# libAudioFlux/audioFlux

Measured on AMD Instinct MI355X. Metric: audio frames/sec (mel+MFCC, n_fft=2048 hop=512), higher is better.
Workload: dtype f32

## Files before the change

### audioflux_amd/csrc/hip/afx_melfused.hip

```cpp
#include <hip/hip_runtime.h>

#include <cstdlib>

#include "afx_melplan.h"

namespace {

const AfxMelSize *size_of(int radix2Exp) {
    switch (radix2Exp) {
        case 9: return afx_mel_size512();
        case 10: return afx_mel_size1k();
        case 11: return afx_mel_size2k();
        case 12: return afx_mel_size4k();
        default: return nullptr;
    }
}

void pack_band(const AfxBandPlan *band, int TA, int WP, float *wL, int *meta) {
    for (int l = 0; l < 64; ++l) {
        for (int t = 0; t < band->tapsA; ++t) wL[(size_t)l * WP + t] = band->wA[(size_t)t * 64 + l];
        for (int t = 0; t < band->tapsB; ++t) wL[(size_t)l * WP + TA + t] = band->wB[(size_t)t * 64 + l];
        meta[l] = band->startA[l];
        meta[64 + l] = band->startB[l];
        meta[128 + l] = band->rowA[l];
        meta[192 + l] = band->rowB[l];
        meta[256 + l] = (int)band->segIdx[l];
        meta[320 + l] = (int)band->segIdx[64 + l];
    }
}

}

extern "C" int afxk_melfused_variant(int radix2Exp, int tapsA, int tapsB) {
    const AfxMelSize *s = size_of(radix2Exp);
    if (afxdev_no_fused() || !s) return -1;
    for (int i = 0; i < s->numVariants; ++i)
        if (tapsA <= s->variants[i].tapsA && tapsB <= s->variants[i].tapsB) return i;
    return -1;
}

extern "C" int afxk_melfused_kind(const void *plan) {
    const AfxMelPlan *p = static_cast<const AfxMelPlan *>(plan);
    return !p ? 0 : size_of(p->radix2Exp)->kindBase + (p->split ? 2 : 1);
}

extern "C" void afxk_melfused_destroy(void *plan) {
    AfxMelPlan *p = static_cast<AfxMelPlan *>(plan);
    if (!p) return;
    afxdev_free(p->dTab);
    afxdev_free(p->dMeta);
    free(p);
}

extern "C" int afxk_melfused_create(void **plan, int radix2Exp, const float *hWindow,
                                    const AfxBandPlan *band, void *stream) {
    *plan = nullptr;
    const int variant = afxk_melfused_variant(radix2Exp, band->tapsA, band->tapsB);
    if (variant < 0) return AFX_ERR_UNSUPPORTED;
    const AfxMelSize *s = size_of(radix2Exp);
    const int TA = s->variants[variant].tapsA, TB = s->variants[variant].tapsB;
    const int WP = TA + TB + 4;
    const size_t bytes = (size_t)s->bandOff + (size_t)64 * WP * 4;
    AfxMelPlan *p = static_cast<AfxMelPlan *>(calloc(1, sizeof(AfxMelPlan)));
    float *tab = static_cast<float *>(calloc(bytes, 1));
    if (!p || !tab) {
        free(p);
        free(tab);
        return AFX_ERR_NOMEM;
    }
    p->radix2Exp = radix2Exp;
    p->variant = variant;
    p->num = band->num;
    p->split = band->split;
    s->fill(tab, hWindow);
    int meta[384];
    pack_band(band, TA, WP, tab + s->bandOff / 4, meta);
    int st = afxdev_malloc(reinterpret_cast<void **>(&p->dTab), bytes);
    if (st == AFX_OK) st = afxdev_h2d(p->dTab, tab, bytes, stream);
    if (st == AFX_OK) st = afxdev_malloc(reinterpret_cast<void **>(&p->dMeta), sizeof(meta));
    if (st == AFX_OK) st = afxdev_h2d(p->dMeta, meta, sizeof(meta), stream);
    if (st == AFX_OK) st = afxdev_stream_sync(stream);
    free(tab);
    if (st != AFX_OK) {
        afxk_melfused_destroy(p);
        return st;
    }
    *plan = p;
    return AFX_OK;
}

extern "C" int afxk_melfused_run(void *plan, const AfxMelFusedArgs *a, void *stream) {
    const AfxMelPlan *p = static_cast<const AfxMelPlan *>(plan);
    if (!p) return AFX_ERR_ARG;
    if (a->energy && p->radix2Exp != 11) return AFX_ERR_UNSUPPORTED;
    if (a->specMap > 4) return AFX_ERR_ARG;
    return size_of(p->radix2Exp)->run(p, a, stream);
}
```

### audioflux_amd/csrc/hip/afx_melfused2.hip

```cpp
#include <hip/hip_runtime.h>

#include <cmath>
#include <cstdlib>
#include <cstring>

#include "afx_melplan.h"
#include "afx_melparts.h"
#include "afx_ccblock.h"

#ifdef AFX_V2_NTIN
#define AFX_V2_LOAD(p) __builtin_nontemporal_load(p)
#define AFX_V2_NT true
#else
#define AFX_V2_LOAD(p) (*(p))
#define AFX_V2_NT false
#endif
#ifndef AFX_V2_CCEVERY
#define AFX_V2_CCEVERY 16
#endif
#ifdef AFX_V2_STAMPS
#include <cstdio>
#include <vector>
#endif

namespace {

constexpr int NFFT = 2048;
constexpr int MC = 1024;
constexpr int WAVES = 12;
constexpr int WAVES_CPLX = 12;
__host__ __device__ constexpr int waves_of(bool cplx) { return cplx ? WAVES_CPLX : WAVES; }
constexpr int P1 = 72;
constexpr int PROW_OFF = 5120;
constexpr int PROW_F = 1104;
constexpr int WAVE_LDS = PROW_OFF + PROW_F * 4;
constexpr int CLAIM_LDS = 16;
static_assert(16 * P1 * 8 <= PROW_OFF + 1025 * 4, "exchange image must end before the zero pad");
constexpr int T_WIN = 0;
constexpr int T_TW1 = 8192;
constexpr int T_TW2 = 16384;
constexpr int TW2_PITCH = 144;
constexpr int T_TW3 = 16960;
constexpr int T_BAND = 21056;
__host__ __device__ constexpr int wpitch(int ta, int tb) { return ta + tb + 4; }
__host__ __device__ constexpr int tab_bytes(int ta, int tb) { return T_BAND + 64 * wpitch(ta, tb) * 4; }
constexpr int DCT_PITCH = 36;
__host__ __device__ constexpr int block_lds_bytes(int ta, int tb, bool cc) {
    return tab_bytes(ta, tb) + (cc ? 64 * DCT_PITCH * 4 : 0) + WAVES * WAVE_LDS + CLAIM_LDS;
}

__host__ __device__ constexpr int claim_length(int left, int waves, int minRun) {
    const int g = left / (2 * waves);
    if (left >= 16 * waves) return g >= 16 ? g & ~15 : 16;
    return (g & ~3) > minRun ? g & ~3 : minRun;
}

struct KArgs2 {
    const float *x;
    long long clipStride;
    long long totalFrames;
    int timeLength, hop;
    long long framesPerWg;
    int aligned;
    const float4 *tab;
    const int *meta;
    int specMap, postPow;
    float normValue;
    float *out;
    float *outIm;
    int num;
    const float *dct;
    int ccNum, ccCbrt;
    float *cc;
    float *energy, *rms, *zcr;
    const float *win;
    int binLo, binCount;
    long long outPitch;
    int vecOut;
#ifdef AFX_V2_STAMPS
    unsigned long long *stamps;
#endif
};
#ifdef AFX_V2_STAMPS
constexpr int STAMP_WORDS = 64, STAMP_HEAD = 8;
#endif


#ifndef AFX_PRIO_MASK
#define AFX_PRIO_MASK 0x1E
#endif
#ifndef AFX_PRIO_LEVEL
#define AFX_PRIO_LEVEL 1
#endif
#define MEL_PHASE(p)                                                                                       \
    do {                                                                                                   \
        if (AFX_PRIO_MASK != 0) __builtin_amdgcn_s_setprio(((AFX_PRIO_MASK >> (p)) & 1) ? AFX_PRIO_LEVEL : 0); \
    } while (0)

__device__ __forceinline__ float wave_sum(float v) {
#pragma unroll
    for (int o = 32; o > 0; o >>= 1) v += __shfl_xor(v, o, 64);
    return v;
}

template <int TA, int TB, int SHIFT, bool SPLIT, int CC, bool TEMPORAL, bool CPLX = false, bool STFT = false>
__global__ __launch_bounds__(waves_of(CPLX) * 64, 3) void k_stft_mel_v2(KArgs2 a) {
    constexpr int NWV = waves_of(CPLX);
    static_assert(!(CPLX && (CC || TEMPORAL)), "complex results: the bank only");
    static_assert(!STFT || (TA == 0 && TB == 0 && !SPLIT && CC == 0 && !TEMPORAL && !CPLX), "STFT instantiations: real rows, no bank");
    extern __shared__ __attribute__((aligned(16))) unsigned char smem[];
    const int lane = threadIdx.x & 63;
    const int wave = threadIdx.x >> 6;
    constexpr int WP = wpitch(TA, TB);
    constexpr int TABB = tab_bytes(TA, TB);
    constexpr int DCTB = CC == 1 ? 64 * DCT_PITCH * 4 : 0;
    unsigned char *wreg = smem + TABB + DCTB + wave * WAVE_LDS;
    float *prow = reinterpret_cast<float *>(wreg + PROW_OFF);

    {
        float4 *s4 = reinterpret_cast<float4 *>(smem);
        for (int i = threadIdx.x + (STFT ? T_TW1 / 16 : 0); i < TABB / 16; i += NWV * 64) s4[i] = a.tab[i];
        if constexpr (STFT) {
            v2 *tw = reinterpret_cast<v2 *>(smem + T_WIN);
            const v2 *w2 = reinterpret_cast<const v2 *>(a.win);
            for (int at = threadIdx.x; at < 1024; at += NWV * 64) {
                const int n1 = 2 * (at >> 7) + (at & 1), l = (at & 127) >> 1;
                tw[at] = w2[64 * n1 + l];
            }
        }
        if constexpr (CC == 1) {
            float *tabD = reinterpret_cast<float *>(smem + TABB);
            for (int i = threadIdx.x; i < 64 * 32; i += NWV * 64) {
                const int l = i >> 5, e = i & 31;
                const int fi = l & 15, g = l >> 4;
                tabD[l * DCT_PITCH + e] =
                    fi < a.ccNum ? a.dct[(long long)fi * a.num + 16 * (e >> 2) + 4 * g + (e & 3)] : 0.f;
            }
        }
        for (int i = 1025 + lane; i < PROW_F; i += 64) prow[i] = 0.f;
        if (threadIdx.x == 0) *reinterpret_cast<int *>(smem + TABB + DCTB + NWV * WAVE_LDS) = 0;
    }
    __syncthreads();

    const int k1 = lane >> 2, m2 = lane & 3;
    const unsigned T0 = lds_addr(smem), W0 = lds_addr(wreg);
    const unsigned aWin = T0 + T_WIN + 16 * lane;
    const unsigned aTw2 = T0 + T_TW2 + TW2_PITCH * m2;
    const unsigned aE1w = W0 + 8 * (8 * (k1 >> 1) + 2 * m2 + (k1 & 1));
    const unsigned aE1r = W0 + 576 * k1 + 16 * m2;
    const unsigned aE2w = W0 + 32 * k1 + 16 * ((m2 >> 1) ^ ((k1 >> 3) & 1)) + 8 * (m2 & 1);
    const int b3l = (lane >> 3) & 1;
    const unsigned aAlo = W0 + 32 * lane + 16 * b3l, aAhi = W0 + 32 * lane + 16 * (1 - b3l);
    const int qm0 = lane == 0 ? 128 : 256 - lane, qm1 = 192 - lane;
    const unsigned aB0lo = W0 + 32 * qm0 + 16 * ((qm0 >> 3) & 1), aB0hi = W0 + 32 * qm0 + 16 * (1 - ((qm0 >> 3) & 1));
    const unsigned aB1lo = W0 + 32 * qm1 + 16 * ((qm1 >> 3) & 1), aB1hi = W0 + 32 * qm1 + 16 * (1 - ((qm1 >> 3) & 1));
    const unsigned aT3lo = T0 + T_TW3 + 32 * lane + 16 * b3l, aT3hi = T0 + T_TW3 + 32 * lane + 16 * (1 - b3l);
    const unsigned R = W0 + PROW_OFF;
    const unsigned aP01 = R + 4 * lane;
    const unsigned aP23 = R + 4 * (lane == 0 ? 128 : lane + 512);
    const unsigned aQs1 = R + 4 * (192 - lane);
    const unsigned aQ23 = R + 4 * (lane == 0 ? 640 : 256 - lane);
    const bool lane0 = (lane == 0);

    const int startA = STFT ? 0 : a.meta[lane], startB = STFT ? 0 : a.meta[64 + lane];
    const int rowA = STFT ? -1 : a.meta[128 + lane], rowB = STFT ? -1 : a.meta[192 + lane];
    const unsigned seg0 = SPLIT ? (unsigned)a.meta[256 + lane] : 0u, seg1 = SPLIT ? (unsigned)a.meta[320 + lane] : 0u;
    const unsigned apa = R + 4 * startA, apb = R + 4 * startB;
    const unsigned awr = T0 + T_BAND + 4 * WP * lane;
    const unsigned vRaw = 8u * (unsigned)lane, vLane = 4u * (unsigned)lane;
    const bool okA = rowA >= 0, okB = rowB >= 0;
    const unsigned vRowA = okA ? 4u * (unsigned)rowA : 0u, vRowB = okB ? 4u * (unsigned)rowB : 0u;
    const long long rowPitch = STFT ? a.outPitch : (long long)a.num;

    const long long wgBeg = (long long)blockIdx.x * a.framesPerWg;
    const int wgN = (int)(a.totalFrames - wgBeg < a.framesPerWg ? a.totalFrames - wgBeg : a.framesPerWg);
    const int minRun = wgN >= 4 * NWV ? 4 : wgN > NWV ? (wgN + NWV - 1) / NWV : 1;
    int *claimed = reinterpret_cast<int *>(smem + TABB + DCTB + NWV * WAVE_LDS);
    const int wgClip = (int)(wgBeg / a.timeLength);
    const unsigned wgT = (unsigned)(wgBeg - (long long)wgClip * a.timeLength);
    auto locate = [&](long long fr, int &c, int &tt) {
        const unsigned at = wgT + (unsigned)(fr - wgBeg);
        c = wgClip + (int)(at / (unsigned)a.timeLength);
        tt = (int)(at % (unsigned)a.timeLength);
    };
    auto claim = [&](long long &rb, long long &re) -> bool {
        int s = wgN, l = 0;
        if (lane0) {
            const int left = wgN - __atomic_load_n(claimed, __ATOMIC_RELAXED);
            if (left > 0) {
                l = claim_length(left, NWV, minRun);
                s = __atomic_fetch_add(claimed, l, __ATOMIC_RELAXED);
            }
        }
        s = __builtin_amdgcn_readfirstlane(s);
        l = __builtin_amdgcn_readfirstlane(l);
        if (s >= wgN) return false;
        rb = wgBeg + s;
        re = wgBeg + (s + l < wgN ? s + l : wgN);
        return true;
    };
    int ccN = 0;
#ifdef AFX_V2_STAMPS
    unsigned long long *stamp = a.stamps + ((long long)blockIdx.x * NWV + wave) * STAMP_WORDS;
    int stampN = 0;
// ... 272 lines not shown
                    split_pair(A1, B1, hi2(wlo[s]), pk[s][1], pq[s][1]);
                    split_pair(A2, B2, lo2(whi[s]), pk[s][2], pq[s][2]);
                    split_pair(A3, B3, hi2(whi[s]), pk[s][3], pq[s][3]);
                }
            }
        }
        if constexpr (CPLX) {
            WR2ST_32(aP01 - PROW_OFF, ik[0][0], ik[0][1], 0, 4);
            WR2ST_32(aP23 - PROW_OFF, ik[0][2], ik[0][3], 0, 4);
            WR2ST_32(aP01 - PROW_OFF, ik[1][0], ik[1][1], 1, 5);
            WR2ST_32(aP01 - PROW_OFF, ik[1][2], ik[1][3], 9, 13);
            WR2ST_32(aQs1 - PROW_OFF, iq[0][1], iq[0][0], 9, 13);
            WR2ST_32(aQ23 - PROW_OFF, iq[0][3], iq[0][2], 0, 4);
            WR2ST_32(aQs1 - PROW_OFF, iq[1][3], iq[1][2], 0, 4);
            WR2ST_32(aQs1 - PROW_OFF, iq[1][1], iq[1][0], 8, 12);
            float *prowI = reinterpret_cast<float *>(wreg);
            if (lane0) prowI[512] = i512;
            prowI[1025 + lane] = 0.f;
            if (lane < PROW_F - 1025 - 64) prowI[1025 + 64 + lane] = 0.f;
        }
        WR2ST_32_S(4, aP01, pk[0][0], pk[0][1], 0, 4);
        WR2ST_32_S(4, aP23, pk[0][2], pk[0][3], 0, 4);
        WR2ST_32_S(4, aP01, pk[1][0], pk[1][1], 1, 5);
        WR2ST_32_S(4, aP01, pk[1][2], pk[1][3], 9, 13);
        WR2ST_32_S(4, aQs1, pq[0][1], pq[0][0], 9, 13);
        WR2ST_32_S(4, aQ23, pq[0][3], pq[0][2], 0, 4);
        WR2ST_32_S(4, aQs1, pq[1][3], pq[1][2], 0, 4);
        WR2ST_32_S(4, aQs1, pq[1][1], pq[1][0], 8, 12);
        if (lane0) prow[512] = p512;
        wave_lds_sync();
#pragma unroll
        for (int pass = 0; pass < (CPLX ? 2 : 1); ++pass) {
        const unsigned bpa = (CPLX && pass) ? apa - PROW_OFF : apa, bpb = (CPLX && pass) ? apb - PROW_OFF : apb;
        if (!CPLX && a.specMap) {
            for (int k = lane; k < 1025; k += 64) {
                const float p = prow[k];
                prow[k] = a.specMap == 1 ? sqrtf(p) : powf(p, a.normValue);
            }
            wave_lds_sync();
        }

        if constexpr (STFT) {
            MEL_PHASE(6);
            raw_landed();
            float *orow = a.out + rowOff;
            if (a.vecOut) {
                const float4 *p4 = reinterpret_cast<const float4 *>(prow);
                float4 *o4 = reinterpret_cast<float4 *>(orow);
                float4 q[4];
#pragma unroll
                for (int i = 0; i < 4; ++i) q[i] = p4[lane + 64 * i];
#pragma unroll
                for (int i = 0; i < 4; ++i) o4[lane + 64 * i] = q[i];
                if (lane0) o4[256] = p4[256];
            } else {
                for (int k = lane; k < a.binCount; k += 64) orow[k] = prow[a.binLo + k];
            }
        } else {
        MEL_PHASE(5);
        float accA, accB;
        {
            v2 sA, sB;
            band_stage<TA, TB, 4, CPLX>(awr, bpa, bpb, sA, sB);
            accA = sA.x + sA.y;
            accB = sB.x + sB.y;
        }
        if (!CPLX && !SPLIT && a.postPow) {
            accA = powf(accA, a.normValue);
            accB = powf(accB, a.normValue);
        }
        MEL_PHASE(6);
        if (pass == 0) raw_landed();
        if constexpr (CC != 0 && !SPLIT) {
            if (ccN == AFX_V2_CCEVERY) cc_block(f - AFX_V2_CCEVERY, (rowOff >> 7) - AFX_V2_CCEVERY, AFX_V2_CCEVERY);
        }
        float *const srow = ((CPLX && pass) ? a.outIm : a.out) + rowOff;
        if constexpr (SPLIT) {
            float *part = reinterpret_cast<float *>(wreg + (CPLX ? PROW_F * 4 : 0));
            static_assert(PROW_F * 4 + 129 * 4 <= PROW_OFF, "segment sums must fit between the two rows");
            part[lane] = accA;
            part[64 + lane] = accB;
            if (lane0) part[128] = 0.f;
            wave_lds_sync();
#pragma unroll
            for (int h = 0; h < 2; ++h) {
                const unsigned u = h ? seg1 : seg0;
                float sum = part[u & 255u] + part[(u >> 8) & 255u];
                sum += part[(u >> 16) & 255u];
                sum += part[u >> 24];
                if (!CPLX && a.postPow) sum = powf(sum, a.normValue);
                if (lane + 64 * h < a.num) GST32_S(vLane, sum, srow + 64 * h);
            }
        } else {
            if (okA) GST32_S(vRowA, accA, srow);
            if (okB) GST32_S(vRowB, accB, srow);
        }
        if constexpr (CC != 0) {
            ++ccN;
            if (f + 1 == fEnd || (SPLIT && ccN == 16)) cc_block(f + 1 - ccN, (rowOff >> 7) + 1 - ccN, ccN);
        }
        }
        wave_lds_sync();

        }

#ifdef AFX_V2_STAMPS
        ++stampN;
        if (lane0 && (stampN & 15) == 0 && STAMP_HEAD + (stampN >> 4) <= STAMP_WORDS) stamp[STAMP_HEAD - 1 + (stampN >> 4)] = __builtin_amdgcn_s_memtime();
#endif
        rowOff += rowPitch;
        if (++t == a.timeLength) {
            t = 0;
            ++clip;
        }
    }
    }
#ifdef AFX_V2_STAMPS
    if (lane0) {
        stamp[1] = __builtin_amdgcn_s_memtime();
        stamp[3] = (unsigned long long)stampN;
    }
#endif
}

void fill_tables(float *tab, const float *hWindow) {
    const double PI = 3.14159265358979323846;
    float *win = tab + T_WIN / 4, *tw1 = tab + T_TW1 / 4, *tw2 = tab + T_TW2 / 4, *tw3 = tab + T_TW3 / 4;
    for (int n1 = 0; n1 < 16; ++n1)
// ... 33 lines not shown
    const int asked = e ? atoi(e) : 0;
    const int cus = asked > 0 ? asked : afx_cu_count();
    long long fpw;
    long long blocks = afx_frame_split(total, cus, waves, 1, &fpw);
    *framesPerWg = fpw * waves;
    if (*framesPerWg > (1ll << 30)) {
        *framesPerWg = 1ll << 30;
        blocks = (total + *framesPerWg - 1) / *framesPerWg;
    }
    return blocks;
}

#ifdef AFX_V2_STAMPS
unsigned long long *stamps_begin(long long blocks, int waves) {
    unsigned long long *d = nullptr;
    const size_t n = (size_t)blocks * waves * STAMP_WORDS * 8;
    if (hipMalloc(&d, n) != hipSuccess || hipMemset(d, 0, n) != hipSuccess) return nullptr;
    return d;
}
void stamps_end(unsigned long long *d, long long blocks, int waves, void *stream) {
    const size_t n = (size_t)blocks * waves * STAMP_WORDS;
    std::vector<unsigned long long> h(n);
    (void)hipStreamSynchronize((hipStream_t)stream);
    if (hipMemcpy(h.data(), d, n * 8, hipMemcpyDeviceToHost) == hipSuccess)
        if (const char *name = getenv("AFX_V2_STAMPS_FILE"))
            if (FILE *fp = fopen(name, "wb")) {
                fwrite(h.data(), 8, n, fp);
                fclose(fp);
            }
    (void)hipFree(d);
}
#endif

template <int TA, int TB, int SHIFT, bool SPLIT, int CC, bool TEMPORAL, bool CPLX = false>
int launch_variant(const AfxMelPlan *p, const AfxMelFusedArgs *a, void *stream) {
    const long long total = (long long)a->batch * a->timeLength;
    if (total <= 0) return AFX_OK;
    constexpr int NWV = waves_of(CPLX);
    long long fpg;
    const long long blocks = wg_ranges(total, NWV, &fpg);

    KArgs2 k;
    memset(&k, 0, sizeof(k));
    k.x = a->x;
    k.clipStride = a->clipStride;
    k.totalFrames = total;
    k.timeLength = a->timeLength;
    k.hop = a->hop;
    k.framesPerWg = fpg;
    k.aligned = ((a->clipStride & 1) == 0) && ((a->hop & 1) == 0) && ((reinterpret_cast<uintptr_t>(a->x) & 7) == 0);
    k.tab = reinterpret_cast<const float4 *>(p->dTab);
    k.meta = p->dMeta;
    k.specMap = a->specMap;
    k.postPow = a->postPow;
    k.normValue = a->normValue;
    k.out = a->out;
    k.outIm = a->outIm;
    k.num = p->num;
    k.dct = a->dct;
    k.ccNum = a->ccNum;
    k.ccCbrt = a->ccRectify == 1;
    k.cc = a->cc;
    k.energy = a->energy;
    k.rms = a->rms;
    k.zcr = a->zcr;
    constexpr size_t lds = (size_t)block_lds_bytes(TA, TB, CC == 1);
    static_assert(lds <= 163840, "workgroup LDS budget");
#ifdef AFX_V2_STAMPS
    if (!(k.stamps = stamps_begin(blocks, NWV))) return AFX_ERR_HIP;
#endif
    AFX_LAUNCH_DYN_LDS((k_stft_mel_v2<TA, TB, SHIFT, SPLIT, CC, TEMPORAL, CPLX>), dim3((unsigned)blocks), dim3(NWV * 64), lds, stream, k);
    AFX_LAUNCH_CHECK("k_stft_mel_v2");
#ifdef AFX_V2_STAMPS
    stamps_end(k.stamps, blocks, NWV, stream);
#endif
    return AFX_OK;
}

template <int TA, int TB, bool SPLIT, int CC, bool TEMPORAL>
int launch_hop(const AfxMelPlan *p, const AfxMelFusedArgs *a, void *stream) {
#ifdef AFX_EXPERIMENTS
    if (const char *e = getenv("AFX_EXP_MEL"))
        if (strstr(e, "noshift")) return launch_variant<TA, TB, 0, SPLIT, CC, TEMPORAL>(p, a, stream);
#endif
    switch (a->hop) {
        case 256: return launch_variant<TA, TB, 2, SPLIT, CC, TEMPORAL>(p, a, stream);
        case 512: return launch_variant<TA, TB, 4, SPLIT, CC, TEMPORAL>(p, a, stream);
        case 1024: return launch_variant<TA, TB, 8, SPLIT, CC, TEMPORAL>(p, a, stream);
        default: return launch_variant<TA, TB, 0, SPLIT, CC, TEMPORAL>(p, a, stream);
    }
}

template <int TA, int TB>
int launch(const AfxMelPlan *p, const AfxMelFusedArgs *a, void *stream) {
    const bool cc = a->cc != nullptr, tmp = a->energy != nullptr;
    if (a->specMap >= 3) {
        if (cc || tmp) return AFX_ERR_UNSUPPORTED;
        if (!a->outIm) return AFX_ERR_ARG;
        if (a->hop == 512)
            return p->split ? launch_variant<TA, TB, 4, true, 0, false, true>(p, a, stream)
                            : launch_variant<TA, TB, 4, false, 0, false, true>(p, a, stream);
        return p->split ? launch_variant<TA, TB, 0, true, 0, false, true>(p, a, stream)
                        : launch_variant<TA, TB, 0, false, 0, false, true>(p, a, stream);
    }
    if (cc && tmp) return AFX_ERR_UNSUPPORTED;
    if (cc) {
        if (a->ccNum < 1 || a->ccNum > 16 || !a->dct || !a->out || p->num > 128 || (p->num & 3)) return AFX_ERR_UNSUPPORTED;
        if (a->ccRectify != 0 && a->ccRectify != 1) return AFX_ERR_UNSUPPORTED;
        if constexpr (block_lds_bytes(TA, TB, true) <= 163840)
            if (!p->split && p->num == 128 && a->ccRectify == 0) return launch_hop<TA, TB, false, 1, false>(p, a, stream);
        if (a->hop == 512)
            return p->split ? launch_variant<TA, TB, 4, true, 2, false>(p, a, stream) : launch_variant<TA, TB, 4, false, 2, false>(p, a, stream);
        return p->split ? launch_variant<TA, TB, 0, true, 2, false>(p, a, stream) : launch_variant<TA, TB, 0, false, 2, false>(p, a, stream);
    }
    if (tmp) {
        if (!a->rms || !a->zcr) return AFX_ERR_ARG;
        return p->split ? launch_hop<TA, TB, true, 0, true>(p, a, stream)
                        : launch_hop<TA, TB, false, 0, true>(p, a, stream);
    }
    return p->split ? launch_hop<TA, TB, true, 0, false>(p, a, stream)
                    : launch_hop<TA, TB, false, 0, false>(p, a, stream);
}

int run(const AfxMelPlan *p, const AfxMelFusedArgs *a, void *stream) {
    return p->variant == 0 ? launch<48, 16>(p, a, stream) : launch<72, 32>(p, a, stream);
}

void fill_stft_tables(float *tab) { fill_tables(tab, nullptr); }

template <int SHIFT>
int launch_stft2k(const AfxStftArgs *a, const float *tab, void *stream) {
    const long long total = (long long)a->batch * a->timeLength;
    long long fpg;
    const long long blocks = wg_ranges(total, WAVES, &fpg);
    KArgs2 k;
    memset(&k, 0, sizeof(k));
    k.x = a->x;
    k.clipStride = a->clipStride;
    k.totalFrames = total;
    k.timeLength = a->timeLength;
    k.hop = a->hop;
    k.framesPerWg = fpg;
    k.aligned = ((a->clipStride & 1) == 0) && ((a->hop & 1) == 0) && ((reinterpret_cast<uintptr_t>(a->x) & 7) == 0);
    k.tab = reinterpret_cast<const float4 *>(tab);
    k.specMap = a->mode == AFX_SPEC_POWER ? 0 : a->mode == AFX_SPEC_MAG ? 1 : 2;
    k.normValue = a->normValue;
    k.out = a->outRe;
    k.win = a->window;
    k.binLo = a->binLo;
    k.binCount = a->binCount;
    k.outPitch = a->outPitch ? a->outPitch : (long long)a->binCount;
    k.vecOut = a->binLo == 0 && a->binCount == NFFT / 2 + 1 && k.outPitch >= 1028 && (k.outPitch & 3) == 0 &&
               (reinterpret_cast<uintptr_t>(a->outRe) & 15) == 0;
    constexpr size_t lds = (size_t)block_lds_bytes(0, 0, false);
#ifdef AFX_V2_STAMPS
    if (!(k.stamps = stamps_begin(blocks, WAVES))) return AFX_ERR_HIP;
#endif
    AFX_LAUNCH_DYN_LDS((k_stft_mel_v2<0, 0, SHIFT, false, 0, false, false, true>), dim3((unsigned)blocks), dim3(WAVES * 64), lds, stream, k);
    AFX_LAUNCH_CHECK("k_stft_mel_v2 (stft)");
#ifdef AFX_V2_STAMPS
    stamps_end(k.stamps, blocks, WAVES, stream);
#endif
    return AFX_OK;
}

}

const AfxMelSize *afx_mel_size2k() {
    static const AfxMelSize size = {11, 0, kVariants, 2, T_BAND, fill_tables, run};
    return &size;
}

extern "C" int afxk_stft2k(const AfxStftArgs *a, void *stream) {
    if (a->radix2Exp != 11 || a->bandStart || a->energy || a->padLeft != 0 || a->hop < 1 || a->binLo < 0 || a->binCount < 1 ||
        a->binLo + a->binCount > NFFT / 2 + 1 || (long long)(a->timeLength - 1) * a->hop + NFFT > a->dataLength ||
        (reinterpret_cast<uintptr_t>(a->window) & 7) != 0)
        return AFX_ERR_UNSUPPORTED;
    if (a->mode != AFX_SPEC_POWER && a->mode != AFX_SPEC_MAG && a->mode != AFX_SPEC_POWER_NORM) return AFX_ERR_UNSUPPORTED;
    if (!a->outRe) return AFX_ERR_ARG;
    const long long total = (long long)a->batch * a->timeLength;
    if (total <= 0) return AFX_OK;
    if (total > 0x7fffffffLL) return AFX_ERR_UNSUPPORTED;
    const float *tab = afx_device_table<fill_stft_tables>((size_t)tab_bytes(0, 0));
    if (!tab) return AFX_ERR_UNSUPPORTED;
    switch (a->hop) {
        case 256: return launch_stft2k<2>(a, tab, stream);
        case 512: return launch_stft2k<4>(a, tab, stream);
        case 1024: return launch_stft2k<8>(a, tab, stream);
        default: return launch_stft2k<0>(a, tab, stream);
    }
}
```

### audioflux_amd/csrc/hip/afx_melparts.h

```cpp
#ifndef AFX_MELPARTS_H
#define AFX_MELPARTS_H

#include <hip/hip_runtime.h>

#include "afx_device.h"
#include "afx_pkmath.h"
#include "afx_frameops.h"

typedef float v4f __attribute__((ext_vector_type(4)));
__device__ __forceinline__ v2 lo2(v4f q) { return v2{q.x, q.y}; }
__device__ __forceinline__ v2 hi2(v4f q) { return v2{q.z, q.w}; }

__device__ __forceinline__ void wave_lds_sync() {
    __builtin_amdgcn_s_waitcnt(0xc07f);
    __builtin_amdgcn_wave_barrier();
}

__device__ __forceinline__ void split_pair(v2 A, v2 B, v2 w, float &pk, float &pq) {
    const v2 e2 = pk_add_conj(A, B);
    const v2 d = pk_sub_conj(A, B);
    const v2 wo = cmul_mi(d, w);
    const v2 p = pair_power(e2, wo);
    pk = p.x;
    pq = p.y;
// ... 70 lines not shown
    for (int blk = 0; blk < NB; ++blk) {
        const int cur = blk & 1;
        const int nextQuads = (blk + 1 < NB) ? ((QT - (blk + 1) * BLK) < BLK ? (QT - (blk + 1) * BLK) : BLK) : 0;
        if (blk + 1 < NB) request(blk + 1, w[cur ^ 1], p0[cur ^ 1], p1[cur ^ 1]);
        if (nextQuads == 4) LDS_WAIT_N(12);
        else if (nextQuads == 3) LDS_WAIT_N(9);
        else if (nextQuads == 2) LDS_WAIT_N(6);
        else if (nextQuads == 1) LDS_WAIT_N(3);
        else LDS_WAIT_N(0);
#pragma unroll
        for (int i = 0; i < BLK; ++i) {
            const int q = blk * BLK + i;
            if (q >= QT) continue;
            PIN(w[cur][i]);
            PIN(p0[cur][i]);
            PIN(p1[cur][i]);
            if (KO_ON(6)) {
                asm volatile("" ::"v"(w[cur][i]), "v"(p0[cur][i]), "v"(p1[cur][i]));
            } else if (q < QA) {
                sA += lo2(w[cur][i]) * p0[cur][i];
                sA += hi2(w[cur][i]) * p1[cur][i];
            } else {
                sB += lo2(w[cur][i]) * p0[cur][i];
                sB += hi2(w[cur][i]) * p1[cur][i];
            }
        }
        if constexpr (PINSUMS) {
            PIN(sA);
            PIN(sB);
        }
    }
}

#endif
```

### audioflux_amd/csrc/hip/afx_melplan.h

```cpp
#ifndef AFX_MELPLAN_H
#define AFX_MELPLAN_H

#include "afx_hipcheck.h"

struct AfxMelPlan {
    int radix2Exp;
    int variant;
    int num;
    int split;
    float *dTab;
    int *dMeta;
};

struct AfxMelVariant {
    int tapsA, tapsB;
};

struct AfxMelSize {
    int radix2Exp;
    int kindBase;
    const AfxMelVariant *variants;
    int numVariants;
    int bandOff;
    void (*fill)(float *tab, const float *hWindow);
    int (*run)(const AfxMelPlan *p, const AfxMelFusedArgs *a, void *stream);
};
const AfxMelSize *afx_mel_size512(), *afx_mel_size1k(), *afx_mel_size2k(), *afx_mel_size4k();

static inline long long afx_mel_frames(long long total, int waves, long long *framesPerWave) {
    return afx_frame_split(total, afx_cu_count(), waves, 2, framesPerWave);
}

#endif
```

### audioflux_amd/csrc/host/afx_bandplan.c

```c
#include <stdlib.h>
#include <string.h>

#include "afx_device.h"
#include "afx_host.h"

typedef struct {
    int row, start, len;
} RowBand;

static int cmp_len_desc(const void *a, const void *b) {
    const RowBand *x = (const RowBand *)a, *y = (const RowBand *)b;
    if (x->len != y->len) return y->len - x->len;
    return x->row - y->row;
}

void afx_bandplan_free(AfxBandPlan *p) {
    if (!p) return;
    free(p->wA);
    free(p->wB);
    p->wA = p->wB = NULL;
}

static int shift_for(const RowBand *r, int residue) {
    int d = (r->start - 2 * residue) % 64;
// ... 217 lines not shown
            p->startA[l] = 2 * (l & 31);
            p->startB[l] = 2 * (l & 31);
            if (nA && laneA[l] >= 0) {
                const RowBand *g = &segA[laneA[l]];
                for (int t = 0; t < g->len; t++)
                    p->wA[(size_t)(t + shiftA[l]) * 64 + l] = bank[(size_t)g->row * F + g->start + t];
                p->startA[l] = g->start - shiftA[l];
                slotOfA[laneA[l]] = l;
            }
            if (nB && laneB[l] >= 0) {
                const RowBand *g = &segB[laneB[l]];
                for (int t = 0; t < g->len; t++)
                    p->wB[(size_t)(t + shiftB[l]) * 64 + l] = bank[(size_t)g->row * F + g->start + t];
                p->startB[l] = g->start - shiftB[l];
                slotOfB[laneB[l]] = l;
            }
        }
        for (int m = 0; m < 128; m++) {
            unsigned packed = 0;
            for (int c = 0; c < 4; c++) {
                unsigned slot = 128;
                if (m < num && c < segCnt[m])
                    slot = segType[m][c] ? 64u + (unsigned)slotOfB[segOf[m][c]] : (unsigned)slotOfA[segOf[m][c]];
                packed |= slot << (8 * c);
            }
            p->segIdx[m] = packed;
        }
    }
    free(rb);
    free(segA);
    free(segB);
    return ok ? 0 : 1;
}
```

Baseline: 710.6 million.

## Pack mel filter rows into three-partition chains to cut band taps

Adds a host-side packer that trims each mel filter row to its nonzero span and packs the 128 rows into per-lane chains across three tap partitions (24/12/12), where a row may continue across partitions. The kernel gets a three-partition band stage with carried partial sums and a third output row per lane. The aim is fewer LDS reads and FMAs per frame than the 48+16 two-set layout, with bank-conflict scoring in the packer. In exchange it adds a randomized search at plan creation, another template instantiation, and a larger metadata table.

After: 729.0 million (median of 6 runs). 2.6% higher.

```diff
diff --git a/audioflux_amd/csrc/hip/afx_melfused.hip b/audioflux_amd/csrc/hip/afx_melfused.hip
--- a/audioflux_amd/csrc/hip/afx_melfused.hip
+++ b/audioflux_amd/csrc/hip/afx_melfused.hip
@@ -3,6 +3,7 @@
 #include <cstdlib>
 
 #include "afx_melplan.h"
+#include "afx_bandpack.h"
 
 namespace {
 
@@ -29,7 +30,21 @@
     }
 }
 
+void pack_band3(const AfxBandPack *pk, int WP, float *wL, int *meta) {
+    for (int l = 0; l < 64; ++l) {
+        for (int t = 0; t < pk->slots; ++t) wL[(size_t)l * WP + t] = pk->w[(size_t)t * 64 + l];
+        for (int q = 0; q < 3; ++q) {
+            meta[64 * q + l] = pk->base[q][l];
+            meta[192 + 64 * q + l] = pk->row[q][l];
+        }
+        meta[384 + l] = pk->cont[1][l];
+        meta[448 + l] = pk->cont[2][l];
+    }
 }
+
+}
+
+extern "C" int afxk_melfused_pack(const void *plan) { return plan ? static_cast<const AfxMelPlan *>(plan)->pack : 0; }
 
 extern "C" int afxk_melfused_variant(int radix2Exp, int tapsA, int tapsB) {
     const AfxMelSize *s = size_of(radix2Exp);
@@ -59,26 +74,43 @@
     if (variant < 0) return AFX_ERR_UNSUPPORTED;
     const AfxMelSize *s = size_of(radix2Exp);
     const int TA = s->variants[variant].tapsA, TB = s->variants[variant].tapsB;
-    const int WP = TA + TB + 4;
+    AfxBandPack pk = {};
+    int pack = 0;
+    const char *nopack = getenv("AFX_MEL_NOPACK");
+    if (s->numPacks > 0 && variant == 0 && !(nopack && atoi(nopack) != 0) &&
+        afx_bandpack_build(band, s->packs, s->numPacks, s->rowCap, TA + TB, &pk) == 0) {
+        for (int i = 0; i < s->numPacks; ++i)
+            if (s->packs[i][0] == pk.taps[0] && s->packs[i][1] == pk.taps[1] && s->packs[i][2] == pk.taps[2]) pack = i + 1;
+        if (!pack) afx_bandpack_free(&pk);
+    }
+    const int WP = (pack ? pk.slots : TA + TB) + 4;
     const size_t bytes = (size_t)s->bandOff + (size_t)64 * WP * 4;
     AfxMelPlan *p = static_cast<AfxMelPlan *>(calloc(1, sizeof(AfxMelPlan)));
     float *tab = static_cast<float *>(calloc(bytes, 1));
     if (!p || !tab) {
         free(p);
         free(tab);
+        if (pack) afx_bandpack_free(&pk);
         return AFX_ERR_NOMEM;
     }
     p->radix2Exp = radix2Exp;
     p->variant = variant;
     p->num = band->num;
     p->split = band->split;
+    p->pack = pack;
     s->fill(tab, hWindow);
-    int meta[384];
-    pack_band(band, TA, WP, tab + s->bandOff / 4, meta);
+    int meta[512];
+    const size_t metaBytes = (pack ? 512 : 384) * sizeof(int);
+    if (pack) {
+        pack_band3(&pk, WP, tab + s->bandOff / 4, meta);
+        afx_bandpack_free(&pk);
+    } else {
+        pack_band(band, TA, WP, tab + s->bandOff / 4, meta);
+    }
     int st = afxdev_malloc(reinterpret_cast<void **>(&p->dTab), bytes);
     if (st == AFX_OK) st = afxdev_h2d(p->dTab, tab, bytes, stream);
-    if (st == AFX_OK) st = afxdev_malloc(reinterpret_cast<void **>(&p->dMeta), sizeof(meta));
-    if (st == AFX_OK) st = afxdev_h2d(p->dMeta, meta, sizeof(meta), stream);
+    if (st == AFX_OK) st = afxdev_malloc(reinterpret_cast<void **>(&p->dMeta), metaBytes);
+    if (st == AFX_OK) st = afxdev_h2d(p->dMeta, meta, metaBytes, stream);
     if (st == AFX_OK) st = afxdev_stream_sync(stream);
     free(tab);
     if (st != AFX_OK) {
diff --git a/audioflux_amd/csrc/hip/afx_melfused2.hip b/audioflux_amd/csrc/hip/afx_melfused2.hip
--- a/audioflux_amd/csrc/hip/afx_melfused2.hip
+++ b/audioflux_amd/csrc/hip/afx_melfused2.hip
@@ -42,11 +42,11 @@
 constexpr int TW2_PITCH = 144;
 constexpr int T_TW3 = 16960;
 constexpr int T_BAND = 21056;
-__host__ __device__ constexpr int wpitch(int ta, int tb) { return ta + tb + 4; }
-__host__ __device__ constexpr int tab_bytes(int ta, int tb) { return T_BAND + 64 * wpitch(ta, tb) * 4; }
+__host__ __device__ constexpr int wpitch(int ta, int tb, int pc = 0) { return ta + tb + pc + 4; }
+__host__ __device__ constexpr int tab_bytes(int ta, int tb, int pc = 0) { return T_BAND + 64 * wpitch(ta, tb, pc) * 4; }
 constexpr int DCT_PITCH = 36;
-__host__ __device__ constexpr int block_lds_bytes(int ta, int tb, bool cc) {
-    return tab_bytes(ta, tb) + (cc ? 64 * DCT_PITCH * 4 : 0) + WAVES * WAVE_LDS + CLAIM_LDS;
+__host__ __device__ constexpr int block_lds_bytes(int ta, int tb, bool cc, int pc = 0) {
+    return tab_bytes(ta, tb, pc) + (cc ? 64 * DCT_PITCH * 4 : 0) + WAVES * WAVE_LDS + CLAIM_LDS;
 }
 
 __host__ __device__ constexpr int claim_length(int left, int waves, int minRun) {
@@ -103,16 +103,17 @@
     return v;
 }
 
-template <int TA, int TB, int SHIFT, bool SPLIT, int CC, bool TEMPORAL, bool CPLX = false, bool STFT = false>
+template <int TA, int TB, int SHIFT, bool SPLIT, int CC, bool TEMPORAL, bool CPLX = false, bool STFT = false, int PC = 0>
 __global__ __launch_bounds__(waves_of(CPLX) * 64, 3) void k_stft_mel_v2(KArgs2 a) {
     constexpr int NWV = waves_of(CPLX);
     static_assert(!(CPLX && (CC || TEMPORAL)), "complex results: the bank only");
     static_assert(!STFT || (TA == 0 && TB == 0 && !SPLIT && CC == 0 && !TEMPORAL && !CPLX), "STFT instantiations: real rows, no bank");
+    static_assert(PC == 0 || (!SPLIT && !STFT), "packed plans hold whole rows");
     extern __shared__ __attribute__((aligned(16))) unsigned char smem[];
     const int lane = threadIdx.x & 63;
     const int wave = threadIdx.x >> 6;
-    constexpr int WP = wpitch(TA, TB);
-    constexpr int TABB = tab_bytes(TA, TB);
+    constexpr int WP = wpitch(TA, TB, PC);
+    constexpr int TABB = tab_bytes(TA, TB, PC);
     constexpr int DCTB = CC == 1 ? 64 * DCT_PITCH * 4 : 0;
     unsigned char *wreg = smem + TABB + DCTB + wave * WAVE_LDS;
     float *prow = reinterpret_cast<float *>(wreg + PROW_OFF);
@@ -162,14 +163,16 @@
     const unsigned aQ23 = R + 4 * (lane == 0 ? 640 : 256 - lane);
     const bool lane0 = (lane == 0);
 
-    const int startA = STFT ? 0 : a.meta[lane], startB = STFT ? 0 : a.meta[64 + lane];
-    const int rowA = STFT ? -1 : a.meta[128 + lane], rowB = STFT ? -1 : a.meta[192 + lane];
+    constexpr int MROW = PC ? 192 : 128;
+    const int startA = STFT ? 0 : a.meta[lane], startB = STFT ? 0 : a.meta[64 + lane], startC = PC ? a.meta[128 + lane] : 0;
+    const int rowA = STFT ? -1 : a.meta[MROW + lane], rowB = STFT ? -1 : a.meta[MROW + 64 + lane], rowC = PC ? a.meta[MROW + 128 + lane] : -1;
     const unsigned seg0 = SPLIT ? (unsigned)a.meta[256 + lane] : 0u, seg1 = SPLIT ? (unsigned)a.meta[320 + lane] : 0u;
-    const unsigned apa = R + 4 * startA, apb = R + 4 * startB;
+    const bool contB = PC ? a.meta[384 + lane] != 0 : false, contC = PC ? a.meta[448 + lane] != 0 : false;
+    const unsigned apa = R + 4 * startA, apb = R + 4 * startB, apc = R + 4 * startC;
     const unsigned awr = T0 + T_BAND + 4 * WP * lane;
     const unsigned vRaw = 8u * (unsigned)lane, vLane = 4u * (unsigned)lane;
-    const bool okA = rowA >= 0, okB = rowB >= 0;
-    const unsigned vRowA = okA ? 4u * (unsigned)rowA : 0u, vRowB = okB ? 4u * (unsigned)rowB : 0u;
+    const bool okA = rowA >= 0, okB = rowB >= 0, okC = rowC >= 0;
+    const unsigned vRowA = okA ? 4u * (unsigned)rowA : 0u, vRowB = okB ? 4u * (unsigned)rowB : 0u, vRowC = okC ? 4u * (unsigned)rowC : 0u;
     const long long rowPitch = STFT ? a.outPitch : (long long)a.num;
 
     const long long wgBeg = (long long)blockIdx.x * a.framesPerWg;
@@ -508,6 +511,7 @@
 #pragma unroll
         for (int pass = 0; pass < (CPLX ? 2 : 1); ++pass) {
         const unsigned bpa = (CPLX && pass) ? apa - PROW_OFF : apa, bpb = (CPLX && pass) ? apb - PROW_OFF : apb;
+        const unsigned bpc = (CPLX && pass) ? apc - PROW_OFF : apc;
         if (!CPLX && a.specMap) {
             for (int k = lane; k < 1025; k += 64) {
                 const float p = prow[k];
@@ -534,8 +538,14 @@
             }
         } else {
         MEL_PHASE(5);
-        float accA, accB;
-        {
+        float accA, accB, accC = 0.f;
+        if constexpr (PC > 0) {
+            v2 sA, sB, sC;
+            band_stage3<TA, TB, PC, 4, CPLX>(awr, bpa, bpb, bpc, contB, contC, sA, sB, sC);
+            accA = sA.x + sA.y;
+            accB = sB.x + sB.y;
+            accC = sC.x + sC.y;
+        } else {
             v2 sA, sB;
             band_stage<TA, TB, 4, CPLX>(awr, bpa, bpb, sA, sB);
             accA = sA.x + sA.y;
@@ -544,6 +554,7 @@
         if (!CPLX && !SPLIT && a.postPow) {
             accA = powf(accA, a.normValue);
             accB = powf(accB, a.normValue);
+            if constexpr (PC > 0) accC = powf(accC, a.normValue);
         }
         MEL_PHASE(6);
         if (pass == 0) raw_landed();
@@ -570,6 +581,9 @@
         } else {
             if (okA) GST32_S(vRowA, accA, srow);
             if (okB) GST32_S(vRowB, accB, srow);
+            if constexpr (PC > 0) {
+                if (okC) GST32_S(vRowC, accC, srow);
+            }
         }
         if constexpr (CC != 0) {
             ++ccN;
@@ -669,7 +683,7 @@
 }
 #endif
 
-template <int TA, int TB, int SHIFT, bool SPLIT, int CC, bool TEMPORAL, bool CPLX = false>
+template <int TA, int TB, int SHIFT, bool SPLIT, int CC, bool TEMPORAL, bool CPLX = false, int PC = 0>
 int launch_variant(const AfxMelPlan *p, const AfxMelFusedArgs *a, void *stream) {
     const long long total = (long long)a->batch * a->timeLength;
     if (total <= 0) return AFX_OK;
@@ -701,12 +715,12 @@
     k.energy = a->energy;
     k.rms = a->rms;
     k.zcr = a->zcr;
-    constexpr size_t lds = (size_t)block_lds_bytes(TA, TB, CC == 1);
+    constexpr size_t lds = (size_t)block_lds_bytes(TA, TB, CC == 1, PC);
     static_assert(lds <= 163840, "workgroup LDS budget");
 #ifdef AFX_V2_STAMPS
     if (!(k.stamps = stamps_begin(blocks, NWV))) return AFX_ERR_HIP;
 #endif
-    AFX_LAUNCH_DYN_LDS((k_stft_mel_v2<TA, TB, SHIFT, SPLIT, CC, TEMPORAL, CPLX>), dim3((unsigned)blocks), dim3(NWV * 64), lds, stream, k);
+    AFX_LAUNCH_DYN_LDS((k_stft_mel_v2<TA, TB, SHIFT, SPLIT, CC, TEMPORAL, CPLX, false, PC>), dim3((unsigned)blocks), dim3(NWV * 64), lds, stream, k);
     AFX_LAUNCH_CHECK("k_stft_mel_v2");
 #ifdef AFX_V2_STAMPS
     stamps_end(k.stamps, blocks, NWV, stream);
@@ -714,17 +728,17 @@
     return AFX_OK;
 }
 
-template <int TA, int TB, bool SPLIT, int CC, bool TEMPORAL>
+template <int TA, int TB, bool SPLIT, int CC, bool TEMPORAL, int PC = 0>
 int launch_hop(const AfxMelPlan *p, const AfxMelFusedArgs *a, void *stream) {
 #ifdef AFX_EXPERIMENTS
     if (const char *e = getenv("AFX_EXP_MEL"))
-        if (strstr(e, "noshift")) return launch_variant<TA, TB, 0, SPLIT, CC, TEMPORAL>(p, a, stream);
+        if (strstr(e, "noshift")) return launch_variant<TA, TB, 0, SPLIT, CC, TEMPORAL, false, PC>(p, a, stream);
 #endif
     switch (a->hop) {
-        case 256: return launch_variant<TA, TB, 2, SPLIT, CC, TEMPORAL>(p, a, stream);
-        case 512: return launch_variant<TA, TB, 4, SPLIT, CC, TEMPORAL>(p, a, stream);
-        case 1024: return launch_variant<TA, TB, 8, SPLIT, CC, TEMPORAL>(p, a, stream);
-        default: return launch_variant<TA, TB, 0, SPLIT, CC, TEMPORAL>(p, a, stream);
+        case 256: return launch_variant<TA, TB, 2, SPLIT, CC, TEMPORAL, false, PC>(p, a, stream);
+        case 512: return launch_variant<TA, TB, 4, SPLIT, CC, TEMPORAL, false, PC>(p, a, stream);
+        case 1024: return launch_variant<TA, TB, 8, SPLIT, CC, TEMPORAL, false, PC>(p, a, stream);
+        default: return launch_variant<TA, TB, 0, SPLIT, CC, TEMPORAL, false, PC>(p, a, stream);
     }
 }
 
@@ -759,7 +773,35 @@
                     : launch_hop<TA, TB, false, 0, false>(p, a, stream);
 }
 
+template <int PA, int PB, int PC>
+int launch_packed(const AfxMelPlan *p, const AfxMelFusedArgs *a, void *stream) {
+    const bool cc = a->cc != nullptr, tmp = a->energy != nullptr;
+    if (a->specMap >= 3) {
+        if (cc || tmp) return AFX_ERR_UNSUPPORTED;
+        if (!a->outIm) return AFX_ERR_ARG;
+        if (a->hop == 512) return launch_variant<PA, PB, 4, false, 0, false, true, PC>(p, a, stream);
+        return launch_variant<PA, PB, 0, false, 0, false, true, PC>(p, a, stream);
+    }
+    if (cc && tmp) return AFX_ERR_UNSUPPORTED;
+    if (cc) {
+        if (a->ccNum < 1 || a->ccNum > 16 || !a->dct || !a->out || p->num > 128 || (p->num & 3)) return AFX_ERR_UNSUPPORTED;
+        if (a->ccRectify != 0 && a->ccRectify != 1) return AFX_ERR_UNSUPPORTED;
+        static_assert(block_lds_bytes(PA, PB, true, PC) <= 163840, "the headline form: DCT operand in LDS");
+        if (p->num == 128 && a->ccRectify == 0) return launch_hop<PA, PB, false, 1, false, PC>(p, a, stream);
+        if (a->hop == 512) return launch_variant<PA, PB, 4, false, 2, false, false, PC>(p, a, stream);
+        return launch_variant<PA, PB, 0, false, 2, false, false, PC>(p, a, stream);
+    }
+    if (tmp) {
+        if (!a->rms || !a->zcr) return AFX_ERR_ARG;
+        return launch_hop<PA, PB, false, 0, true, PC>(p, a, stream);
+    }
+    return launch_hop<PA, PB, false, 0, false, PC>(p, a, stream);
+}
+
+constexpr int kPacks[][3] = {{24, 12, 12}};
+
 int run(const AfxMelPlan *p, const AfxMelFusedArgs *a, void *stream) {
+    if (p->pack == 1) return launch_packed<24, 12, 12>(p, a, stream);
     return p->variant == 0 ? launch<48, 16>(p, a, stream) : launch<72, 32>(p, a, stream);
 }
 
@@ -804,7 +846,7 @@
 }
 
 const AfxMelSize *afx_mel_size2k() {
-    static const AfxMelSize size = {11, 0, kVariants, 2, T_BAND, fill_tables, run};
+    static const AfxMelSize size = {11, 0, kVariants, 2, T_BAND, fill_tables, run, kPacks, 1, PROW_F};
     return &size;
 }
 
diff --git a/audioflux_amd/csrc/hip/afx_melparts.h b/audioflux_amd/csrc/hip/afx_melparts.h
--- a/audioflux_amd/csrc/hip/afx_melparts.h
+++ b/audioflux_amd/csrc/hip/afx_melparts.h
@@ -126,4 +126,74 @@
     }
 }
 
+template <int PA, int PB, int PC, int BLK, bool PINSUMS>
+__device__ __forceinline__ void band_stage3(unsigned awr, unsigned ap0, unsigned ap1, unsigned ap2, bool cont1, bool cont2, v2 &s0, v2 &s1,
+                                            v2 &s2) {
+    constexpr int Q0 = PA / 4, Q1 = Q0 + PB / 4, QT = Q1 + PC / 4, NB = (QT + BLK - 1) / BLK;
+    static_assert(BLK <= 4, "the wait ladder counts up to four quads in flight");
+    static_assert(PA % 4 == 0 && PB % 4 == 0 && PC % 4 == 0 && PA > 0 && PB > 0 && PC > 0, "partitions are whole quads");
+    s0 = v2{0.f, 0.f};
+    s1 = v2{0.f, 0.f};
+    s2 = v2{0.f, 0.f};
+    v4f w[2][BLK];
+    v2 p0[2][BLK], p1[2][BLK];
+    auto request = [&](int blk, v4f (&wq)[BLK], v2 (&q0v)[BLK], v2 (&q1v)[BLK]) {
+#pragma unroll
+        for (int i = 0; i < BLK; ++i) {
+            const int q = blk * BLK + i;
+            if (q >= QT) continue;
+            RD128_S(3, wq[i], awr, 16 * q);
+            if (q < Q0) {
+                RD64_S(3, q0v[i], ap0, 16 * q);
+                RD64_S(3, q1v[i], ap0, 16 * q + 8);
+            } else if (q < Q1) {
+                RD64_S(3, q0v[i], ap1, 16 * (q - Q0));
+                RD64_S(3, q1v[i], ap1, 16 * (q - Q0) + 8);
+            } else {
+                RD64_S(3, q0v[i], ap2, 16 * (q - Q1));
+                RD64_S(3, q1v[i], ap2, 16 * (q - Q1) + 8);
+            }
+        }
+    };
+    request(0, w[0], p0[0], p1[0]);
+#pragma unroll
+    for (int blk = 0; blk < NB; ++blk) {
+        const int cur = blk & 1;
+        const int nextQuads = (blk + 1 < NB) ? ((QT - (blk + 1) * BLK) < BLK ? (QT - (blk + 1) * BLK) : BLK) : 0;
+        if (blk + 1 < NB) request(blk + 1, w[cur ^ 1], p0[cur ^ 1], p1[cur ^ 1]);
+        if (nextQuads == 4) LDS_WAIT_N(12);
+        else if (nextQuads == 3) LDS_WAIT_N(9);
+        else if (nextQuads == 2) LDS_WAIT_N(6);
+        else if (nextQuads == 1) LDS_WAIT_N(3);
+        else LDS_WAIT_N(0);
+#pragma unroll
+        for (int i = 0; i < BLK; ++i) {
+            const int q = blk * BLK + i;
+            if (q >= QT) continue;
+            PIN(w[cur][i]);
+            PIN(p0[cur][i]);
+            PIN(p1[cur][i]);
+            if (q == Q0) s1 = cont1 ? s0 : v2{0.f, 0.f};
+            if (q == Q1) s2 = cont2 ? s1 : v2{0.f, 0.f};
+            if (KO_ON(6)) {
+                asm volatile("" ::"v"(w[cur][i]), "v"(p0[cur][i]), "v"(p1[cur][i]));
+            } else if (q < Q0) {
+                s0 += lo2(w[cur][i]) * p0[cur][i];
+                s0 += hi2(w[cur][i]) * p1[cur][i];
+            } else if (q < Q1) {
+                s1 += lo2(w[cur][i]) * p0[cur][i];
+                s1 += hi2(w[cur][i]) * p1[cur][i];
+            } else {
+                s2 += lo2(w[cur][i]) * p0[cur][i];
+                s2 += hi2(w[cur][i]) * p1[cur][i];
+            }
+        }
+        if constexpr (PINSUMS) {
+            PIN(s0);
+            PIN(s1);
+            PIN(s2);
+        }
+    }
+}
+
 #endif
diff --git a/audioflux_amd/csrc/hip/afx_melplan.h b/audioflux_amd/csrc/hip/afx_melplan.h
--- a/audioflux_amd/csrc/hip/afx_melplan.h
+++ b/audioflux_amd/csrc/hip/afx_melplan.h
@@ -8,6 +8,7 @@
     int variant;
     int num;
     int split;
+    int pack;
     float *dTab;
     int *dMeta;
 };
@@ -24,8 +25,13 @@
     int bandOff;
     void (*fill)(float *tab, const float *hWindow);
     int (*run)(const AfxMelPlan *p, const AfxMelFusedArgs *a, void *stream);
+    const int (*packs)[3];
+    int numPacks;
+    int rowCap;
 };
 const AfxMelSize *afx_mel_size512(), *afx_mel_size1k(), *afx_mel_size2k(), *afx_mel_size4k();
+
+extern "C" int afxk_melfused_pack(const void *plan);
 
 static inline long long afx_mel_frames(long long total, int waves, long long *framesPerWave) {
     return afx_frame_split(total, afx_cu_count(), waves, 2, framesPerWave);
diff --git a/audioflux_amd/csrc/host/afx_bandpack.h b/audioflux_amd/csrc/host/afx_bandpack.h
--- /dev/null
+++ b/audioflux_amd/csrc/host/afx_bandpack.h
@@ -0,0 +1,29 @@
+#ifndef AFX_BANDPACK_H
+#define AFX_BANDPACK_H
+
+#include "afx_device.h"
+
+#ifdef __cplusplus
+extern "C" {
+#endif
+
+typedef struct {
+    int num;
+    int taps[3];
+    int slots;
+    int conflicts;
+    int base[3][64];
+    int row[3][64];
+    int cont[3][64];
+    float *w;
+} AfxBandPack;
+
+#define AFX_BANDPACK_MAX_PAIRS 1
+int afx_bandpack_build(const AfxBandPlan *plan, const int (*layouts)[3], int n, int rowCap, int curSlots, AfxBandPack *out);
+void afx_bandpack_free(AfxBandPack *p);
+
+#ifdef __cplusplus
+}
+#endif
+
+#endif
diff --git a/audioflux_amd/csrc/host/afx_bandplan.c b/audioflux_amd/csrc/host/afx_bandplan.c
--- a/audioflux_amd/csrc/host/afx_bandplan.c
+++ b/audioflux_amd/csrc/host/afx_bandplan.c
@@ -273,3 +273,289 @@
     free(segB);
     return ok ? 0 : 1;
 }
+
+#include "afx_bandpack.h"
+
+typedef struct {
+    int row;
+    int start, len;
+    int set, lane, t0;
+    unsigned char d[32];
+} PackRow;
+
+typedef struct {
+    int first, parts, cap;
+    int key;
+    int idx;
+    int r;
+    int lane, base;
+} PackChain;
+
+static unsigned pack_rand(unsigned *s) {
+    *s = (unsigned)(((unsigned long long)*s * 1664525ull + 1013904223ull) & 0xffffffffull);
+    return *s >> 8;
+}
+
+static int pack_need(const PackRow *r) { return r->row < 0 ? 0 : r->len + (r->start & 1); }
+
+static int cmp_need_desc(const void *a, const void *b) {
+    const PackRow *x = (const PackRow *)a, *y = (const PackRow *)b;
+    const int nx = pack_need(x), ny = pack_need(y);
+    if (nx != ny) return ny - nx;
+    return x->row - y->row;
+}
+
+static int cmp_cap_desc(const void *a, const void *b) {
+    const PackChain *x = (const PackChain *)a, *y = (const PackChain *)b;
+    if (x->cap != y->cap) return y->cap - x->cap;
+    if (x->key != y->key) return x->key - y->key;
+    return x->idx - y->idx;
+}
+
+static int chain_base(const PackChain *c, const PackRow *r, int residue, int rowCap) {
+    if (r->row < 0) return 2 * residue;
+    const int d = r->d[residue];
+    if (d > r->start || r->len + d > c->cap || r->start - d + c->cap > rowCap) return -1;
+    return r->start - d;
+}
+
+static int kuhn_try(int u, int m, char adj[64][64], int *owner, char *seen, int rot) {
+    for (int k = 0; k < m; k++) {
+        const int s = (k + rot) % m;
+        if (!adj[u][s] || seen[s]) continue;
+        seen[s] = 1;
+        if (owner[s] < 0 || kuhn_try(owner[s], m, adj, owner, seen, rot)) {
+            owner[s] = u;
+            return 1;
+        }
+    }
+    return 0;
+}
+
+static int pack_stage(PackChain *ch, const PackRow *rows, const int *list, int n, const int *slotHalf, const int *slotRes, int m,
+                      int openLane[2][32], const int *nOpen, int rowCap, unsigned *seed) {
+    char adj[64][64];
+    int owner[64], used[2] = {0, 0}, slotOf[64];
+    for (int u = 0; u < n; u++)
+        for (int s = 0; s < m; s++) adj[u][s] = chain_base(&ch[list[u]], &rows[ch[list[u]].r], slotRes[s], rowCap) >= 0;
+    for (int s = 0; s < m; s++) owner[s] = -1;
+    for (int u = 0; u < n; u++) slotOf[u] = -1;
+    const int rot = m ? (int)(pack_rand(seed) % (unsigned)m) : 0;
+    for (int u = 0; u < n; u++) {
+        char seen[64];
+        memset(seen, 0, sizeof(seen));
+        kuhn_try(u, m, adj, owner, seen, rot);
+    }
+    for (int s = 0; s < m; s++)
+        if (owner[s] >= 0) slotOf[owner[s]] = s;
+    for (int u = 0; u < n; u++) {
+        if (slotOf[u] < 0) continue;
+        PackChain *c = &ch[list[u]];
+        const int h = slotHalf[slotOf[u]];
+        if (used[h] >= nOpen[h]) return 1;
+        c->lane = openLane[h][used[h]++];
+        c->base = chain_base(c, &rows[c->r], slotRes[slotOf[u]], rowCap);
+    }
+    for (int u = 0; u < n; u++) {
+        if (slotOf[u] >= 0) continue;
+        PackChain *c = &ch[list[u]];
+        const PackRow *r = &rows[c->r];
+        const int h = used[0] < nOpen[0] ? 0 : 1;
+        if (used[h] >= nOpen[h]) return 1;
+        c->lane = openLane[h][used[h]++];
+        c->base = r->start - (r->start & 1);
+        if (c->base + c->cap > rowCap) return 1;
+    }
+    return 0;
+}
+
+static int pack_conflicts(int base[3][64]) {
+    int pairs = 0;
+    for (int p = 0; p < 3; p++)
+        for (int h = 0; h < 2; h++) {
+            int cnt[32];
+            memset(cnt, 0, sizeof(cnt));
+            for (int l = 32 * h; l < 32 * h + 32; l++) cnt[(base[p][l] / 2) & 31]++;
+            for (int r = 0; r < 32; r++) pairs += cnt[r] * (cnt[r] - 1) / 2;
+        }
+    return pairs;
+}
+
+static int pack_deal(PackChain *ch, const PackRow *rows, const int *t, int x, int y, int z, unsigned *seed) {
+    const int a = t[0], b = t[1], c = t[2];
+    const int first[6] = {0, 0, 0, 1, 1, 2}, parts[6] = {3, 2, 1, 2, 1, 1};
+    const int cap[6] = {a + b + c, a + b, a, b + c, b, c}, cnt[6] = {x, y, x + z, z, x, x + y};
+    int n = 0;
+    for (int k = 0; k < 6; k++)
+        for (int i = 0; i < cnt[k]; i++, n++) {
+            ch[n].first = first[k], ch[n].parts = parts[k], ch[n].cap = cap[k];
+            ch[n].key = seed ? (int)(pack_rand(seed) & 0xffff) : n;
+            ch[n].idx = n;
+            ch[n].lane = ch[n].base = -1;
+        }
+    qsort(ch, 128, sizeof(PackChain), cmp_cap_desc);
+    for (int i = 0; i < 128; i++) {
+        ch[i].r = i;
+        if (pack_need(&rows[i]) > ch[i].cap) return 0;
+    }
+    if (seed)
+        for (int k = 0; k < 64; k++) {
+            const int i = (int)(pack_rand(seed) % 127u);
+            if (pack_need(&rows[ch[i].r]) <= ch[i + 1].cap && pack_need(&rows[ch[i + 1].r]) <= ch[i].cap) {
+                const int tmp = ch[i].r;
+                ch[i].r = ch[i + 1].r, ch[i + 1].r = tmp;
+            }
+        }
+    return 1;
+}
+
+static int pack_try(PackChain *ch, const PackRow *rows, const int *t, int rowCap, unsigned *seed, int cover[3][64], int base[3][64]) {
+    int list[64], slotHalf[64], slotRes[64], openLane[2][32], nOpen[2];
+    for (int p = 0; p < 3; p++) {
+        int n = 0, m = 0;
+        for (int i = 0; i < 128; i++)
+            if (ch[i].first == p) list[n++] = i;
+        for (int i = n - 1; i > 0; i--) {
+            const int j = (int)(pack_rand(seed) % (unsigned)(i + 1)), tmp = list[i];
+            list[i] = list[j], list[j] = tmp;
+        }
+        for (int h = 0; h < 2; h++) {
+            char busy[32];
+            memset(busy, 0, sizeof(busy));
+            nOpen[h] = 0;
+            for (int l = 32 * h; l < 32 * h + 32; l++) {
+                const int prev = p ? cover[p - 1][l] : -1;
+                if (prev >= 0 && ch[prev].first + ch[prev].parts > p) {
+                    cover[p][l] = prev;
+                    base[p][l] = base[p - 1][l] + t[p - 1];
+                    busy[(base[p][l] / 2) & 31] = 1;
+                } else {
+                    openLane[h][nOpen[h]++] = l;
+                }
+            }
+            int free_ = 0;
+            for (int r = 0; r < 32 && free_ < nOpen[h]; r++)
+                if (!busy[r]) slotHalf[m] = h, slotRes[m] = r, m++, free_++;
+        }
+        if (n != nOpen[0] + nOpen[1] || m < n) return -1;
+        if (pack_stage(ch, rows, list, n, slotHalf, slotRes, m, openLane, nOpen, rowCap, seed)) return -1;
+        for (int i = 0; i < n; i++) {
+            cover[p][ch[list[i]].lane] = list[i];
+            base[p][ch[list[i]].lane] = ch[list[i]].base;
+        }
+    }
+    return pack_conflicts(base);
+}
+
+void afx_bandpack_free(AfxBandPack *p) {
+    if (!p) return;
+    free(p->w);
+    p->w = NULL;
+}
+
+int afx_bandpack_build(const AfxBandPlan *plan, const int (*layouts)[3], int n, int rowCap, int curSlots, AfxBandPack *out) {
+    memset(out, 0, sizeof(*out));
+    if (!plan || plan->split || plan->num <= 64 || plan->num > 128 || !plan->wA || !plan->wB || n < 1) return 1;
+    PackRow rows[128];
+    int nr = 0, longest = 0;
+    for (int set = 0; set < 2; set++)
+        for (int l = 0; l < 64; l++) {
+            const int row = set ? plan->rowB[l] : plan->rowA[l], taps = set ? plan->tapsB : plan->tapsA;
+            const float *w = set ? plan->wB : plan->wA;
+            if (row < 0) continue;
+            if (nr == 128) return 1;
+            int f = -1, last = -1;
+            for (int k = 0; k < taps; k++)
+                if (w[(size_t)k * 64 + l] != 0.f) {
+                    if (f < 0) f = k;
+                    last = k;
+                }
+            PackRow *r = &rows[nr++];
+            r->row = row, r->set = set, r->lane = l;
+            r->t0 = f < 0 ? 0 : f;
+            r->len = f < 0 ? 0 : last - f + 1;
+            r->start = (set ? plan->startB[l] : plan->startA[l]) + r->t0;
+            if (pack_need(r) > longest) longest = pack_need(r);
+        }
+    if (nr != plan->num) return 1;
+    for (; nr < 128; nr++) rows[nr].row = -1, rows[nr].start = rows[nr].len = rows[nr].set = rows[nr].lane = rows[nr].t0 = 0;
+    qsort(rows, 128, sizeof(PackRow), cmp_need_desc);
+    for (int i = 0; i < 128; i++)
+        for (int res = 0; res < 32; res++) rows[i].d[res] = (unsigned char)(((rows[i].start - 2 * res) % 64 + 64) % 64);
+
+    int order[16];
+    if (n > 16) n = 16;
+    for (int i = 0; i < n; i++) order[i] = i;
+    for (int i = 1; i < n; i++)
+        for (int j = i; j > 0; j--) {
+            const int *u = layouts[order[j]], *v = layouts[order[j - 1]];
+            if (u[0] + u[1] + u[2] >= v[0] + v[1] + v[2]) break;
+            const int tmp = order[j];
+            order[j] = order[j - 1], order[j - 1] = tmp;
+        }
+    for (int li = 0; li < n; li++) {
+        const int *t = layouts[order[li]];
+        const int slots = t[0] + t[1] + t[2];
+        if (t[0] < 4 || t[1] < 4 || t[2] < 4 || ((t[0] | t[1] | t[2]) & 3) || slots < longest) continue;
+        if (slots >= curSlots) break;
+        enum { MAXC = 8, TRIES = 48 };
+        int candX[MAXC], candY[MAXC], candS[MAXC], nc = 0;
+        PackChain ch[128];
+        for (int x = 0; x <= 32; x++)
+            for (int y = 0; y <= 64 - 2 * x; y++) {
+                if (!pack_deal(ch, rows, t, x, y, 64 - 2 * x - y, NULL)) continue;
+                int score = 0;
+                for (int i = 0; i < 128; i++) {
+                    const int opt = (ch[i].cap - pack_need(&rows[ch[i].r])) / 2 + 1;
+                    score += opt < 6 ? opt : 6;
+                }
+                int at;
+                if (nc < MAXC) at = nc++;
+                else if (score > candS[MAXC - 1]) at = MAXC - 1;
+                else continue;
+                while (at > 0 && candS[at - 1] < score) {
+                    candX[at] = candX[at - 1], candY[at] = candY[at - 1], candS[at] = candS[at - 1];
+                    at--;
+                }
+                candX[at] = x, candY[at] = y, candS[at] = score;
+            }
+        if (!nc) continue;
+        int best = -1, bestCover[3][64], bestBase[3][64];
+        PackChain bestCh[128];
+        unsigned seed = 2024u;
+        for (int k = 0; k < TRIES * nc && best != 0; k++) {
+            const int ci = k % nc;
+            int cover[3][64], base[3][64];
+            if (!pack_deal(ch, rows, t, candX[ci], candY[ci], 64 - 2 * candX[ci] - candY[ci], k < nc ? NULL : &seed)) continue;
+            const int got = pack_try(ch, rows, t, rowCap, &seed, cover, base);
+            if (got >= 0 && (best < 0 || got < best)) {
+                best = got;
+                memcpy(bestCover, cover, sizeof(cover));
+                memcpy(bestBase, base, sizeof(base));
+                memcpy(bestCh, ch, sizeof(ch));
+            }
+        }
+        if (best < 0 || best > AFX_BANDPACK_MAX_PAIRS) continue;
+        out->w = (float *)calloc((size_t)slots * 64, sizeof(float));
+        if (!out->w) return 1;
+        out->num = plan->num;
+        out->taps[0] = t[0], out->taps[1] = t[1], out->taps[2] = t[2];
+        out->slots = slots;
+        out->conflicts = best;
+        const int off[3] = {0, t[0], t[0] + t[1]};
+        for (int l = 0; l < 64; l++)
+            for (int p = 0; p < 3; p++) {
+                const PackChain *c = &bestCh[bestCover[p][l]];
+                const PackRow *r = &rows[c->r];
+                out->base[p][l] = bestBase[p][l];
+                out->cont[p][l] = c->first < p;
+                out->row[p][l] = c->first + c->parts - 1 == p ? r->row : -1;
+                if (c->first != p || r->row < 0) continue;
+                const float *w = r->set ? plan->wB : plan->wA;
+                const int d = r->start - c->base;
+                for (int k = 0; k < r->len; k++) out->w[(size_t)(off[p] + d + k) * 64 + l] = w[(size_t)(r->t0 + k) * 64 + r->lane];
+            }
+        return 0;
+    }
+    return 1;
+}
```
